# jiangzhengkai/mxdetection

Measured on AMD Instinct MI355X. Metric: images/sec (whole node) Faster R-CNN R50-FPN 3x800x1333, higher is better.
Workload: dtype bf16; 1 GPU; Faster R-CNN ResNet-50-FPN bf16 train step, batch 2/GPU, 3x800x1333 (padded 1344); global_batch=2, parallelism=dp1, frozen=stem+C2, frozen BN folded, optimizer=SGD momentum 0.9 wd 1e-4, launch=hipGraph replay, input=resident, wgrad_side_stream=True, rpn_branch_stream=True, grouped_wgrad=True, filter_prefetch_hints=True, params_trainable=41538304

## Files before the change

### mxdetection_amd/csrc/boxes.hip

```cpp
#include "common.h"

namespace mxdet {

__global__ void box_iou_kernel(const float4* __restrict__ a, int64_t na, const float4* __restrict__ b,
                               int64_t nb, float* __restrict__ out) {
  int64_t idx = (int64_t)blockIdx.x * blockDim.x + threadIdx.x;
  if (idx >= na * nb) return;
  int64_t i = idx / nb, j = idx - i * nb;
  float4 p = a[i], q = b[j];
  out[idx] = mxdet_iou(p.x, p.y, p.z, p.w, q.x, q.y, q.z, q.w);
}

__global__ void anchors_kernel(const float* __restrict__ base, int A, int H, int W, int stride,
                               float4* __restrict__ out) {
  int64_t idx = (int64_t)blockIdx.x * blockDim.x + threadIdx.x;
  int64_t total = (int64_t)H * W * A;
  if (idx >= total) return;
  int a = (int)(idx % A);
  int64_t cell = idx / A;
  int x = (int)(cell % W), y = (int)(cell / W);
  float sx = (float)(x * stride), sy = (float)(y * stride);
  float4 o;
  o.x = base[a * 4 + 0] + sx;
  o.y = base[a * 4 + 1] + sy;
  o.z = base[a * 4 + 2] + sx;
  o.w = base[a * 4 + 3] + sy;
  out[idx] = o;
}

__global__ void fpn_level_kernel(const float* __restrict__ rois, int64_t R, int lvl_min, int lvl_max,
                                 int32_t* __restrict__ levels) {
  int64_t i = (int64_t)blockIdx.x * blockDim.x + threadIdx.x;
  if (i >= R) return;
  const float* r = rois + i * 5;
  int k = mxdet_fpn_level(r[1], r[2], r[3], r[4]);
  k = k < lvl_min ? lvl_min : (k > lvl_max ? lvl_max : k);
  levels[i] = k;
}

__global__ void __launch_bounds__(64)
nms_mask_kernel(const float4* __restrict__ boxes, const int32_t* __restrict__ counts, int n_max,
                int nwords_max, float thresh, unsigned long long* __restrict__ mask) {
  const int col_blk = blockIdx.x, row_blk = blockIdx.y, b = blockIdx.z;
  if (col_blk < row_blk) return;
  int n = counts[b];
  n = n > n_max ? n_max : n;
  if (row_blk * 64 >= n || col_blk * 64 >= n) return;
  __shared__ float4 cb[64];
  const int t = threadIdx.x;
  const float4* bx = boxes + (int64_t)b * n_max;
  int cj = col_blk * 64 + t;
  if (cj < n) cb[t] = bx[cj];
  __syncthreads();
  int i = row_blk * 64 + t;
  if (i >= n) return;
  float4 r = bx[i];
  int ncol = n - col_blk * 64;
  ncol = ncol > 64 ? 64 : ncol;
  unsigned long long bits = 0;
  for (int j = 0; j < ncol; ++j) {
    int c = col_blk * 64 + j;
    float4 q = cb[j];
    float v = mxdet_iou(r.x, r.y, r.z, r.w, q.x, q.y, q.z, q.w);
    if (c > i && v > thresh) bits |= (1ull << j);
  }
  mask[((int64_t)b * n_max + i) * nwords_max + col_blk] = bits;
}

__device__ __forceinline__ unsigned long long readlane64(unsigned long long v, int lane) {
  unsigned lo = (unsigned)v, hi = (unsigned)(v >> 32);
  lo = (unsigned)__builtin_amdgcn_readlane((int)lo, lane);
  hi = (unsigned)__builtin_amdgcn_readlane((int)hi, lane);
  return ((unsigned long long)hi << 32) | lo;
}

__global__ void __launch_bounds__(64)
nms_scan_kernel(const unsigned long long* __restrict__ mask, const int32_t* __restrict__ counts,
                const uint8_t* __restrict__ invalid, int n_max, int nwords_max, int max_keep,
                int32_t* __restrict__ keep_idx, int32_t* __restrict__ num_keep) {
  __shared__ unsigned long long rem[64];
  const int b = blockIdx.x, lane = threadIdx.x;
  int n = counts[b];
  n = n > n_max ? n_max : n;
  n = __builtin_amdgcn_readfirstlane(n);
  const int nw = (n + 63) >> 6;
  const unsigned long long* m = mask + (int64_t)b * n_max * nwords_max;
  for (int w = 0; w < nw; ++w) {
    int idx = w * 64 + lane;
    bool bad = (idx >= n) || (invalid != nullptr && invalid[(int64_t)b * n_max + idx] != 0);
    unsigned long long bm = __ballot(bad);
    if (lane == 0) rem[w] = bm;
  }
  __syncthreads();
  unsigned long long mykeep = 0;
  unsigned long long diag_next = (nw > 0 && lane < n) ? m[(int64_t)lane * nwords_max] : 0ull;
  for (int w = 0; w < nw; ++w) {
    const unsigned long long diag = diag_next;
    if (w + 1 < nw) {
      int row = (w + 1) * 64 + lane;
      diag_next = (row < n) ? m[(int64_t)row * nwords_max + (w + 1)] : 0ull;
    }
    __syncthreads();
    unsigned long long cur = rem[w];
    cur = readlane64(cur, 0);
    unsigned long long keepbits = 0;
    for (int bb = 0; bb < 64; ++bb) {
      unsigned long long d = readlane64(diag, bb);
      if (!((cur >> bb) & 1ull)) {
        keepbits |= (1ull << bb);
        cur |= d;
      }
    }
    if (lane == w) mykeep = keepbits;
    if ((keepbits >> lane) & 1ull) {
      const unsigned long long* row = m + (int64_t)(w * 64 + lane) * nwords_max;
      for (int j = w + 1; j < nw; ++j) {
        unsigned long long v = row[j];
        if (v) atomicOr(&rem[j], v);
      }
    }
  }
  int cnt = __popcll(mykeep);
  int incl = cnt;
  for (int off = 1; off < 64; off <<= 1) {
    int v = __shfl_up(incl, off);
    if (lane >= off) incl += v;
  }
  int excl = incl - cnt;
  int total = __shfl(incl, 63);
  unsigned long long kb = mykeep;
  int pos = excl;
  while (kb) {
    int bb = __ffsll((long long)kb) - 1;
    kb &= kb - 1;
    if (pos < max_keep) keep_idx[(int64_t)b * n_max + pos] = lane * 64 + bb;
    ++pos;
  }
  if (lane == 0) num_keep[b] = total < max_keep ? total : max_keep;
}

template <int NW>
__global__ void __launch_bounds__(64)
nms_scan_rows_kernel(const unsigned long long* __restrict__ mask, const int32_t* __restrict__ counts,
                     const uint8_t* __restrict__ invalid, int n_max, int nwords_max, int max_keep,
                     int32_t* __restrict__ keep_idx, int32_t* __restrict__ num_keep) {
  __shared__ unsigned long long rows[2][64][NW + 1];
  const int b = blockIdx.x, lane = threadIdx.x;
  int n = counts[b];
  n = n > n_max ? n_max : n;
  n = __builtin_amdgcn_readfirstlane(n);
  const int nw = (n + 63) >> 6;
  const unsigned long long* m = mask + (int64_t)b * n_max * NW;
  unsigned long long myrem = 0ull;
  for (int w = 0; w < nw; ++w) {
    int idx = w * 64 + lane;
    bool bad = (idx >= n) || (invalid != nullptr && invalid[(int64_t)b * n_max + idx] != 0);
    unsigned long long bm = __ballot(bad);
    if (lane == w) myrem = bm;
  }
  unsigned long long nxt[NW];
  auto load_row = [&](unsigned long long (&r)[NW], int w) {
    const unsigned long long* bp = m + (int64_t)(w * 64) * NW + lane;
#pragma unroll
    for (int k = 0; k < NW; ++k) r[k] = bp[k * 64];
  };
  auto stage = [&](const unsigned long long (&r)[NW], int buf, int w) {
    unsigned long long* dst = &rows[buf][lane >> 5][lane & 31];
#pragma unroll
    for (int k = 0; k < NW; ++k) dst[k * 2 * (NW + 1)] = r[k];
  };
  load_row(nxt, 0);
  stage(nxt, 0, 0);
  __syncthreads();
  const int myword = lane < NW ? lane : 0;
  unsigned long long mykeep = 0;
  int buf = 0;
  for (int w = 0; w < nw; ++w) {
#ifndef NMS_ABL_NOLOAD
    if (w + 1 < nw) load_row(nxt, w + 1);
#endif
    const unsigned long long diag = rows[buf][lane][w];
    unsigned long long c = readlane64(myrem, w);
#ifndef NMS_ABL_NOCHAIN
#pragma unroll
    for (int bb = 0; bb < 64; ++bb) {
      unsigned long long d = readlane64(diag, bb);
      c |= ((c >> bb) & 1ull) ? 0ull : d;
    }
#else
    c |= readlane64(diag, 0);
#endif
    const unsigned long long keepbits = ~c;
    if (lane == w) mykeep = keepbits;
    const unsigned klo = __builtin_amdgcn_readfirstlane((unsigned)keepbits);
    const unsigned khi = __builtin_amdgcn_readfirstlane((unsigned)(keepbits >> 32));
    unsigned long long acc = 0ull;
#ifndef NMS_ABL_NOOR
#pragma unroll
#else
    if (klo == 0x12345u)
#endif
    for (int ch = 0; ch < 8; ++ch) {
      const unsigned bits = ((ch < 4 ? klo : khi) >> (8 * (ch & 3))) & 0xffu;
      if (bits == 0u) continue;
      unsigned long long v[8];
#pragma unroll
      for (int t = 0; t < 8; ++t) v[t] = rows[buf][8 * ch + t][myword];
#pragma unroll
      for (int t = 0; t < 8; ++t) acc |= ((bits >> t) & 1u) ? v[t] : 0ull;
    }
    if (lane > w && lane < nw) myrem |= acc;
    if (w + 1 < nw) stage(nxt, buf ^ 1, w + 1);
    __syncthreads();
    buf ^= 1;
  }
  int cnt = __popcll(mykeep);
  int incl = cnt;
  for (int off = 1; off < 64; off <<= 1) {
    int v = __shfl_up(incl, off);
    if (lane >= off) incl += v;
  }
  int excl = incl - cnt;
  int total = __shfl(incl, 63);
  unsigned long long kb = mykeep;
  int pos = excl;
  while (kb) {
    int bb = __ffsll((long long)kb) - 1;
    kb &= kb - 1;
    if (pos < max_keep) keep_idx[(int64_t)b * n_max + pos] = lane * 64 + bb;
    ++pos;
  }
  if (lane == 0) num_keep[b] = total < max_keep ? total : max_keep;
}

}

using namespace mxdet;

extern "C" int mxdet_box_iou(const float* boxes_a, int64_t na, const float* boxes_b, int64_t nb,
                             float* out, mxdet_stream_t stream) {
  clear_error();
  MXDET_REQUIRE(na >= 0 && nb >= 0, MXDET_ESHAPE, "box_iou: negative size");
  if (na == 0 || nb == 0) return MXDET_OK;
  MXDET_REQUIRE(boxes_a && boxes_b && out, MXDET_EINVAL, "box_iou: null pointer");
  int64_t total = na * nb;
  hipLaunchKernelGGL(box_iou_kernel, dim3((unsigned)ceil_div<int64_t>(total, 256)), dim3(256), 0,
                     as_stream(stream), (const float4*)boxes_a, na, (const float4*)boxes_b, nb, out);
  return check_launch("box_iou");
}

extern "C" int mxdet_generate_anchors(const float* base_anchors, int32_t A, int32_t H, int32_t W,
                                      int32_t stride, float* out, mxdet_stream_t stream) {
  clear_error();
  MXDET_REQUIRE(A > 0 && H >= 0 && W >= 0 && stride > 0, MXDET_ESHAPE, "generate_anchors: bad shape");
  int64_t total = (int64_t)H * W * A;
  if (total == 0) return MXDET_OK;
  MXDET_REQUIRE(base_anchors && out, MXDET_EINVAL, "generate_anchors: null pointer");
  hipLaunchKernelGGL(anchors_kernel, dim3((unsigned)ceil_div<int64_t>(total, 256)), dim3(256), 0,
                     as_stream(stream), base_anchors, A, H, W, stride, (float4*)out);
  return check_launch("generate_anchors");
}

extern "C" int mxdet_fpn_level_map(const float* rois, int64_t R, int32_t lvl_min, int32_t lvl_max,
                                   int32_t* levels, mxdet_stream_t stream) {
  clear_error();
  MXDET_REQUIRE(R >= 0 && lvl_min <= lvl_max, MXDET_ESHAPE, "fpn_level_map: bad arguments");
  if (R == 0) return MXDET_OK;
  MXDET_REQUIRE(rois && levels, MXDET_EINVAL, "fpn_level_map: null pointer");
  hipLaunchKernelGGL(fpn_level_kernel, dim3((unsigned)ceil_div<int64_t>(R, 256)), dim3(256), 0,
                     as_stream(stream), rois, R, lvl_min, lvl_max, levels);
  return check_launch("fpn_level_map");
}

extern "C" size_t mxdet_nms_batched_workspace_bytes(int32_t B, int32_t n_max) {
  if (B <= 0 || n_max <= 0) return 0;
  size_t nwords = (size_t)(n_max + 63) / 64;
  if (nwords <= 32) nwords = 32;
  return ((size_t)B * n_max + 64) * nwords * sizeof(unsigned long long);
}

extern "C" int mxdet_nms_batched(const float* boxes, const int32_t* counts, const uint8_t* invalid,
                                 int32_t B, int32_t n_max, float thresh, int32_t max_keep,
                                 int32_t* keep_idx, int32_t* num_keep, void* workspace,
                                 size_t workspace_bytes, mxdet_stream_t stream) {
  clear_error();
  MXDET_REQUIRE(B >= 0 && n_max >= 0, MXDET_ESHAPE, "nms_batched: negative size");
  if (B == 0) return MXDET_OK;
  MXDET_REQUIRE(n_max <= 4096, MXDET_ESHAPE, "nms_batched: n_max %d > 4096 unsupported", n_max);
  MXDET_REQUIRE(counts && num_keep, MXDET_EINVAL, "nms_batched: null pointer");
  if (n_max == 0) {
    hipError_t e = zero_async(num_keep, sizeof(int32_t) * B, as_stream(stream));
    MXDET_REQUIRE(e == hipSuccess, MXDET_EHIP, "nms_batched: memset failed");
    return MXDET_OK;
  }
  MXDET_REQUIRE(boxes && keep_idx, MXDET_EINVAL, "nms_batched: null pointer");
  size_t need = mxdet_nms_batched_workspace_bytes(B, n_max);
  MXDET_REQUIRE(workspace && workspace_bytes >= need, MXDET_EWORKSPACE,
                "nms_batched: workspace %zu < %zu", workspace_bytes, need);
  int nwords = (n_max + 63) / 64;
  const int pitch = nwords <= 32 ? 32 : nwords;
  hipLaunchKernelGGL(nms_mask_kernel, dim3(nwords, nwords, B), dim3(64), 0, as_stream(stream),
                     (const float4*)boxes, counts, n_max, pitch, thresh,
                     (unsigned long long*)workspace);
  if (nwords <= 32)
    hipLaunchKernelGGL(nms_scan_rows_kernel<32>, dim3(B), dim3(64), 0, as_stream(stream),
                       (const unsigned long long*)workspace, counts, invalid, n_max, nwords,
                       max_keep < 0 ? 0 : max_keep, keep_idx, num_keep);
  else
    hipLaunchKernelGGL(nms_scan_kernel, dim3(B), dim3(64), 0, as_stream(stream),
                       (const unsigned long long*)workspace, counts, invalid, n_max, nwords,
                       max_keep < 0 ? 0 : max_keep, keep_idx, num_keep);
  return check_launch("nms_batched");
}
```

### mxdetection_amd/csrc/proposal.hip

```cpp
#include "common.h"
#include "select.h"

namespace mxdet {

constexpr int kMaxPre = 4096;

struct PyramidDev {
  int num_levels, A, dtype;
  int H[8], W[8], stride[8];
  const void* cls[8];
  const void* reg[8];
  long long cls_sn[8], cls_sy[8], cls_sx[8], cls_sa[8];
  long long reg_sn[8], reg_sy[8], reg_sx[8], reg_sc[8];
  const float* base[8];
  long long level_offset[8];
  int classes;
};

__device__ __forceinline__ float pyr_score(const PyramidDev& p, int l, int n, int local) {
  int A = p.A;
  int a = local % A;
  int cell = local / A;
  int x = cell % p.W[l], y = cell / p.W[l];
  long long off = n * p.cls_sn[l] + y * p.cls_sy[l] + x * p.cls_sx[l] + a * p.cls_sa[l];
// ... 40 lines not shown
      wave_scan_bins(sd.hist + ((size_t)ps * sd.B + b) * 256, st.remaining, &bin, &cum, &bc, &tot);
      if (bin == 256) { st.all = 1; break; }
      st.prefix |= (unsigned)bin << shift;
      st.mask |= 255u << shift;
      st.remaining -= cum;
      st.eq_count = bc;
    }
    if (threadIdx.x == 0) *sh = st;
  }
  __syncthreads();
  return *sh;
}

__global__ void __launch_bounds__(256)
proposal_hist_kernel(PyramidDev p, long long A_total, const unsigned* __restrict__ fkeys, SelDev sd, int pass) {
  __shared__ unsigned h[256];
  __shared__ SelState sh;
  const int l = blockIdx.y, n = blockIdx.z;
  const int nl = p.H[l] * p.W[l] * p.A;
  const int c0 = blockIdx.x * kSelChunk;
  if (c0 >= nl) return;
  const int b = n * p.num_levels + l;
  h[threadIdx.x] = 0u;
  SelState st = sel_resolve(sd, b, pass, &sh);
  if (st.all) return;
  const unsigned* fk_l = fkeys + (long long)n * A_total + p.level_offset[l];
  const int shift = 24 - 8 * pass;
  const int c1 = c0 + kSelChunk < nl ? c0 + kSelChunk : nl;
  for (int i0 = c0 + threadIdx.x; i0 < c1; i0 += 4 * 256) {
    unsigned kv[4];
#pragma unroll
    for (int u = 0; u < 4; ++u) {
      int i = i0 + u * 256;
      kv[u] = i < c1 ? (~fk_l[i]) & sd.keymask : 0u;
    }
#pragma unroll
    for (int u = 0; u < 4; ++u)
      hist_add_agg(h, (i0 + u * 256 < c1) && (kv[u] & st.mask) == st.prefix, (kv[u] >> shift) & 255u);
  }
  __syncthreads();
  unsigned v = h[threadIdx.x];
  if (v) atomicAdd(&sd.hist[((size_t)pass * sd.B + b) * 256 + threadIdx.x], v);
}

__global__ void __launch_bounds__(256)
proposal_select_kernel(PyramidDev p, long long A_total, const unsigned* __restrict__ fkeys, SelDev sd,
                       unsigned long long* __restrict__ keys) {
  __shared__ SelState sh;
  const int l = blockIdx.y, n = blockIdx.z;
  const int nl = p.H[l] * p.W[l] * p.A;
  const int c0 = blockIdx.x * kSelChunk;
  if (c0 >= nl) return;
  const int b = n * p.num_levels + l;
  const SelState st = sel_resolve(sd, b, sd.npass, &sh);
  const bool split_ties = !st.all && st.remaining < st.eq_count;
  const unsigned goff = (unsigned)p.level_offset[l];
  const unsigned* fk_l = fkeys + (long long)n * A_total + p.level_offset[l];
  unsigned* ties = sd.ties + (long long)n * A_total + p.level_offset[l];
  unsigned long long* out = keys + (long long)b * sd.pre_n;
  const int c1 = c0 + kSelChunk < nl ? c0 + kSelChunk : nl;
  __shared__ unsigned long long s_take[kSelChunk];
  __shared__ unsigned s_tie[kSelChunk];
  __shared__ int s_nt, s_ni, s_bt, s_bi;
  if (threadIdx.x == 0) { s_nt = 0; s_ni = 0; }
  __syncthreads();
  for (int i = c0 + (int)threadIdx.x; i < c1; i += 256) {
    const unsigned fk = fk_l[i];
    const unsigned kv = (~fk) & sd.keymask;
    if (st.all || kv < st.prefix || (kv == st.prefix && !split_ties))
      s_take[atomicAdd(&s_nt, 1)] = ((unsigned long long)fk << 32) | (unsigned long long)(0xffffffffu - (goff + (unsigned)i));
    else if (split_ties && kv == st.prefix)
      s_tie[atomicAdd(&s_ni, 1)] = (unsigned)i;
  }
  __syncthreads();
  if (threadIdx.x == 0) {
    s_bt = s_nt ? atomicAdd(&sd.cnt[b * 2 + 0], s_nt) : 0;
    s_bi = s_ni ? atomicAdd(&sd.cnt[b * 2 + 1], s_ni) : 0;
  }
  __syncthreads();
  for (int j = threadIdx.x; j < s_nt; j += 256) out[s_bt + j] = s_take[j];
  for (int j = threadIdx.x; j < s_ni; j += 256) ties[s_bi + j] = s_tie[j];
}

__global__ void __launch_bounds__(1024)
proposal_finish_kernel(PyramidDev p, long long A_total, const unsigned* __restrict__ fkeys, SelDev sd, int Kpad,
                       unsigned long long* __restrict__ keys, int32_t* __restrict__ counts) {
  __shared__ SelectSmem sm;
  __shared__ SelState sh;
  __shared__ unsigned long long list[kMaxPre];
  __shared__ int n_sel;
  const int l = blockIdx.x, n = blockIdx.y;
  const int b = n * p.num_levels + l;
  const SelState st = sel_resolve(sd, b, sd.npass, &sh);
  const bool split_ties = !st.all && st.remaining < st.eq_count;
  const int got = sd.cnt[b * 2 + 0], n_tie = sd.cnt[b * 2 + 1];
  unsigned long long* out = keys + (long long)b * sd.pre_n;
  for (int i = threadIdx.x; i < Kpad; i += blockDim.x) list[i] = i < got ? out[i] : 0ull;
  if (threadIdx.x == 0) n_sel = got;
  __syncthreads();
  if (split_ties) {
    const unsigned goff = (unsigned)p.level_offset[l];
    const unsigned* fk_l = fkeys + (long long)n * A_total + p.level_offset[l];
    const unsigned* ties = sd.ties + (long long)n * A_total + p.level_offset[l];
    const unsigned T = st.prefix;
    auto tkey = [&](int, unsigned& kv) -> bool { kv = T; return true; };
    auto tidx = [&](int i) -> unsigned { return ties[i]; };
    const unsigned IT = block_tie_threshold(n_tie, st.remaining, T, tkey, tidx, sm);
    for (int j = threadIdx.x; j < n_tie; j += blockDim.x) {
      unsigned i = ties[j];
      if (i <= IT) {
        int pos = atomicAdd(&n_sel, 1);
        list[pos] = ((unsigned long long)fk_l[i] << 32) | (unsigned long long)(0xffffffffu - (goff + i));
      }
    }
    __syncthreads();
  }
  block_bitonic_sort_desc(list, Kpad);
  const int cnt = n_sel;
  for (int i = threadIdx.x; i < sd.pre_n; i += blockDim.x) out[i] = list[i];
  if (threadIdx.x == 0) counts[b] = cnt;
}

__global__ void proposal_decode_kernel(PyramidDev p, int N, int pre_n, const float* __restrict__ im_info,
                                       float min_size, const unsigned long long* __restrict__ keys,
                                       const int32_t* __restrict__ counts, float4* __restrict__ boxes,
                                       uint8_t* __restrict__ invalid) {
  int idx = blockIdx.x * blockDim.x + threadIdx.x;
  int B = N * p.num_levels;
  if (idx >= B * pre_n) return;
  int b = idx / pre_n, j = idx - b * pre_n;
  int n = b / p.num_levels, l = b - n * p.num_levels;
  if (j >= counts[b]) {
    boxes[idx] = make_float4(0.f, 0.f, 0.f, 0.f);
    invalid[idx] = 1;
    return;
  }
  unsigned long long key = keys[idx];
  unsigned gidx = 0xffffffffu - (unsigned)(key & 0xffffffffull);
  int local = (int)(gidx - (unsigned)p.level_offset[l]);
  int A = p.A;
  int a = local % A;
  int cell = local / A;
  int x = cell % p.W[l], y = cell / p.W[l];
  a /= p.classes;
  const float* base = p.base[l] + a * 4;
  float sx = (float)(x * p.stride[l]), sy = (float)(y * p.stride[l]);
  float ax1 = base[0] + sx, ay1 = base[1] + sy, ax2 = base[2] + sx, ay2 = base[3] + sy;
  long long off = n * p.reg_sn[l] + y * p.reg_sy[l] + x * p.reg_sx[l];
  float d0 = load_as_f32(p.reg[l], off + (a * 4 + 0) * p.reg_sc[l], p.dtype);
  float d1 = load_as_f32(p.reg[l], off + (a * 4 + 1) * p.reg_sc[l], p.dtype);
  float d2 = load_as_f32(p.reg[l], off + (a * 4 + 2) * p.reg_sc[l], p.dtype);
  float d3 = load_as_f32(p.reg[l], off + (a * 4 + 3) * p.reg_sc[l], p.dtype);
  float o[4];
  mxdet_decode_clip(ax1, ay1, ax2, ay2, d0, d1, d2, d3, im_info[n * 3 + 0], im_info[n * 3 + 1], o);
  float ms = min_size * im_info[n * 3 + 2];
  float w = o[2] - o[0] + 1.0f, h = o[3] - o[1] + 1.0f;
  boxes[idx] = make_float4(o[0], o[1], o[2], o[3]);
  invalid[idx] = (w < ms || h < ms) ? 1 : 0;
}

__global__ void __launch_bounds__(1024)
proposal_merge_kernel(int L, int pre_n, int lvl_cap, int post_n,
                      const unsigned long long* __restrict__ keys,
                      const float4* __restrict__ boxes, const int32_t* __restrict__ keep_idx,
                      const int32_t* __restrict__ num_keep, float* __restrict__ rois,
                      float* __restrict__ roi_scores, int32_t* __restrict__ roi_anchor,
                      int32_t* __restrict__ num_rois) {
  extern __shared__ __attribute__((aligned(16))) unsigned char smem_raw[];
  unsigned long long* lk = (unsigned long long*)smem_raw;
  __shared__ int nk[8];
  const int n = blockIdx.y, l_own = blockIdx.x;
  if (threadIdx.x < L) {
    int v = num_keep[n * L + threadIdx.x];
    nk[threadIdx.x] = v > lvl_cap ? lvl_cap : v;
  }
  __syncthreads();
  int total = 0;
  for (int l = 0; l < L; ++l) total += nk[l];
  for (int l = 0; l < L; ++l) {
    int b = n * L + l;
    for (int j = threadIdx.x; j < nk[l]; j += blockDim.x)
      lk[l * lvl_cap + j] = keys[(long long)b * pre_n + keep_idx[(long long)b * pre_n + j]];
  }
  __syncthreads();
  {
    const int l = l_own;
    int b = n * L + l;
    for (int j = threadIdx.x; j < nk[l]; j += blockDim.x) {
      unsigned long long e = lk[l * lvl_cap + j];
      int rank = j;
      for (int l2 = 0; l2 < L; ++l2) {
        if (l2 == l) continue;
        int lo = 0, hi = nk[l2];
        const unsigned long long* q = lk + l2 * lvl_cap;
        while (lo < hi) {
          int mid = (lo + hi) >> 1;
          if (q[mid] > e) lo = mid + 1; else hi = mid;
        }
        rank += lo;
      }
      if (rank < post_n) {
        int pos = keep_idx[(long long)b * pre_n + j];
        float4 bx = boxes[(long long)b * pre_n + pos];
        float* r = rois + ((long long)n * post_n + rank) * 5;
        r[0] = (float)n; r[1] = bx.x; r[2] = bx.y; r[3] = bx.z; r[4] = bx.w;
        unsigned fk = (unsigned)(e >> 32);
        unsigned u = (fk & 0x80000000u) ? (fk & 0x7fffffffu) : ~fk;
        roi_scores[(long long)n * post_n + rank] = __uint_as_float(u);
        roi_anchor[(long long)n * post_n + rank] = (int32_t)(0xffffffffu - (unsigned)(e & 0xffffffffull));
      }
    }
  }
  if (l_own != 0) return;
  int nout = total < post_n ? total : post_n;
  for (int j = nout + threadIdx.x; j < post_n; j += blockDim.x) {
    float* r = rois + ((long long)n * post_n + j) * 5;
    r[0] = (float)n; r[1] = 0.f; r[2] = 0.f; r[3] = 0.f; r[4] = 0.f;
    roi_scores[(long long)n * post_n + j] = 0.f;
    roi_anchor[(long long)n * post_n + j] = -1;
  }
  if (threadIdx.x == 0) num_rois[n] = nout;
}

struct ProposalWs {
  unsigned* fkeys;
  unsigned* hist;
  int* cnt;
  unsigned* ties;
  unsigned long long* keys;
  int32_t* counts;
  float4* boxes;
  uint8_t* invalid;
  int32_t* keep_idx;
  int32_t* num_keep;
  void* nms_ws;
  size_t nms_bytes;
  size_t total;
};

static ProposalWs carve(void* base, int B, int pre_n, int N, long long A_total) {
  ProposalWs w;
// ... 18 lines not shown
  w.nms_ws = (void*)(p + take(w.nms_bytes));
  w.total = off;
  return w;
}

}

using namespace mxdet;

extern "C" size_t mxdet_proposal_workspace_bytes(const mxdet_pyramid_t* p, int32_t N,
                                                 int32_t pre_nms_top_n) {
  if (!p || N <= 0 || pre_nms_top_n <= 0 || p->num_levels <= 0) return 0;
  long long At = 0;
  for (int l = 0; l < p->num_levels; ++l) At += (long long)p->H[l] * p->W[l] * p->A;
  return carve(nullptr, N * p->num_levels, pre_nms_top_n, N, At).total;
}

extern "C" int mxdet_proposal(const mxdet_pyramid_t* p, int32_t N, const float* im_info,
                              int32_t pre_nms_top_n, int32_t post_nms_top_n, float nms_thresh,
                              float min_size, float* rois, float* roi_scores, int32_t* roi_anchor,
                              int32_t* num_rois, void* workspace, size_t workspace_bytes,
                              mxdet_stream_t stream) {
  clear_error();
  MXDET_REQUIRE(p != nullptr, MXDET_EINVAL, "proposal: null pyramid");
  MXDET_REQUIRE(N > 0 && p->num_levels > 0 && p->num_levels <= 8 && p->A > 0, MXDET_ESHAPE,
                "proposal: bad N/levels/A");
  MXDET_REQUIRE(pre_nms_top_n > 0 && pre_nms_top_n <= kMaxPre, MXDET_ESHAPE,
                "proposal: pre_nms_top_n %d outside (0,%d]", pre_nms_top_n, kMaxPre);
  MXDET_REQUIRE(post_nms_top_n > 0 && post_nms_top_n <= pre_nms_top_n * p->num_levels, MXDET_ESHAPE,
                "proposal: bad post_nms_top_n %d", post_nms_top_n);
  MXDET_REQUIRE(p->dtype == MXDET_DTYPE_F32 || p->dtype == MXDET_DTYPE_BF16, MXDET_EINVAL,
                "proposal: bad dtype");
  MXDET_REQUIRE(im_info && rois && roi_scores && roi_anchor && num_rois, MXDET_EINVAL,
                "proposal: null pointer");
  const int L = p->num_levels, B = N * L;
  long long A_total = 0;
  for (int l = 0; l < L; ++l) A_total += (long long)p->H[l] * p->W[l] * p->A;
  ProposalWs w = carve(workspace, B, pre_nms_top_n, N, A_total);
  MXDET_REQUIRE(workspace && workspace_bytes >= w.total, MXDET_EWORKSPACE,
                "proposal: workspace %zu < %zu", workspace_bytes, w.total);
  int per_level_post = post_nms_top_n < pre_nms_top_n ? post_nms_top_n : pre_nms_top_n;
  size_t merge_lds = (size_t)L * per_level_post * 8;
  MXDET_REQUIRE(merge_lds <= 150 * 1024, MXDET_ESHAPE, "proposal: levels*post_nms_top_n too large");
  PyramidDev d;
  memset(&d, 0, sizeof(d));
  d.num_levels = L; d.A = p->A; d.dtype = p->dtype;
  d.classes = p->classes > 1 ? p->classes : 1;
  MXDET_REQUIRE(p->A % d.classes == 0, MXDET_ESHAPE, "proposal: A=%d is not a multiple of classes=%d", p->A, d.classes);
  long long off = 0;
  for (int l = 0; l < L; ++l) {
    MXDET_REQUIRE(p->H[l] > 0 && p->W[l] > 0 && p->stride[l] > 0 && p->cls[l] && p->reg[l] &&
                      p->base_anchors[l],
                  MXDET_EINVAL, "proposal: level %d incomplete", l);
    MXDET_REQUIRE((long long)p->H[l] * p->W[l] * p->A < (1ll << 30), MXDET_ESHAPE,
                  "proposal: level %d too large", l);
    d.H[l] = p->H[l]; d.W[l] = p->W[l]; d.stride[l] = p->stride[l];
    d.cls[l] = p->cls[l]; d.reg[l] = p->reg[l];
    d.cls_sn[l] = p->cls_sn[l]; d.cls_sy[l] = p->cls_sy[l]; d.cls_sx[l] = p->cls_sx[l]; d.cls_sa[l] = p->cls_sa[l];
    d.reg_sn[l] = p->reg_sn[l]; d.reg_sy[l] = p->reg_sy[l]; d.reg_sx[l] = p->reg_sx[l]; d.reg_sc[l] = p->reg_sc[l];
    d.base[l] = p->base_anchors[l];
    d.level_offset[l] = off;
    off += (long long)p->H[l] * p->W[l] * p->A;
  }
  int Kpad = 1;
  while (Kpad < pre_nms_top_n) Kpad <<= 1;
  hipStream_t s = as_stream(stream);
  SelDev sd;
  sd.hist = w.hist; sd.cnt = w.cnt; sd.ties = w.ties;
  sd.npass = (p->dtype == MXDET_DTYPE_BF16) ? 2 : 4;
  sd.keymask = (p->dtype == MXDET_DTYPE_BF16) ? 0xffff0000u : 0xffffffffu;
  sd.B = B; sd.pre_n = pre_nms_top_n;
  int max_nl = 0;
  for (int l = 0; l < L; ++l) max_nl = max_nl > p->H[l] * p->W[l] * p->A ? max_nl : p->H[l] * p->W[l] * p->A;
  long long gthreads = (long long)N * A_total;
  if (gthreads < (long long)kMaxPasses * B * 256) gthreads = (long long)kMaxPasses * B * 256;
  hipLaunchKernelGGL(proposal_gather_kernel, dim3((unsigned)ceil_div<long long>(gthreads, 256)), dim3(256), 0, s, d,
                     N, A_total, w.fkeys, sd);
  const dim3 sel_grid(ceil_div(max_nl, kSelChunk), L, N);
  for (int ps = 0; ps < sd.npass; ++ps)
    hipLaunchKernelGGL(proposal_hist_kernel, sel_grid, dim3(256), 0, s, d, A_total, (const unsigned*)w.fkeys, sd, ps);
  hipLaunchKernelGGL(proposal_select_kernel, sel_grid, dim3(256), 0, s, d, A_total, (const unsigned*)w.fkeys, sd,
                     w.keys);
  hipLaunchKernelGGL(proposal_finish_kernel, dim3(L, N), dim3(1024), 0, s, d, A_total, (const unsigned*)w.fkeys, sd,
                     Kpad, w.keys, w.counts);
  int tot = B * pre_nms_top_n;
  hipLaunchKernelGGL(proposal_decode_kernel, dim3(ceil_div(tot, 256)), dim3(256), 0, s, d, N,
                     pre_nms_top_n, im_info, min_size, w.keys, w.counts, w.boxes, w.invalid);
  int rc = check_launch("proposal(topk/decode)");
  if (rc) return rc;
  rc = mxdet_nms_batched((const float*)w.boxes, w.counts, w.invalid, B, pre_nms_top_n, nms_thresh,
                         per_level_post, w.keep_idx, w.num_keep, w.nms_ws, w.nms_bytes, stream);
  if (rc) return rc;
  hipLaunchKernelGGL(proposal_merge_kernel, dim3(L, N), dim3(1024), merge_lds, s, L, pre_nms_top_n,
                     per_level_post, post_nms_top_n, w.keys, w.boxes, w.keep_idx, w.num_keep, rois, roi_scores,
                     roi_anchor, num_rois);
  return check_launch("proposal(merge)");
}
```

### mxdetection_amd/csrc/targets.hip

```cpp
#include "common.h"
#include "select.h"

namespace mxdet {

__global__ void __launch_bounds__(256)
anchor_iou_kernel(const float4* __restrict__ anchors, long long A_total, const float* __restrict__ gt,
                  int G_max, const float* __restrict__ im_info, float allowed_border,
                  float* __restrict__ max_iou, int32_t* __restrict__ argmax,
                  unsigned* __restrict__ gt_max) {
  extern __shared__ __attribute__((aligned(16))) unsigned char smem_raw[];
  float* sg = (float*)smem_raw;
  unsigned* sgm = (unsigned*)(sg + G_max * 5);
  const int n = blockIdx.y;
  for (int i = threadIdx.x; i < G_max * 5; i += blockDim.x) sg[i] = gt[(long long)n * G_max * 5 + i];
  for (int i = threadIdx.x; i < G_max; i += blockDim.x) sgm[i] = 0u;
  __syncthreads();
  long long a = (long long)blockIdx.x * blockDim.x + threadIdx.x;
  if (a < A_total) {
    float4 b = anchors[a];
    float im_h = im_info[n * 3 + 0], im_w = im_info[n * 3 + 1];
    bool inside = (b.x >= -allowed_border) && (b.y >= -allowed_border) &&
                  (b.z < im_w + allowed_border) && (b.w < im_h + allowed_border);
    float best = -1.0f;
    int bi = -1;
// ... 118 lines not shown
  if (inside) {
    key = mxdet_sample_key(seed, step, image_offset + (unsigned)n, 1u, (unsigned)a);
    labels[(long long)n * A_total + a] = 0;
    max_iou[(long long)n * A_total + a] = 0.0f;
    keys[(long long)n * A_total + a] = key;
  }
  if (cand.count != nullptr) cand_append(cand, n, inside ? 0 : -1, key, (int)a);
}

struct AnchorSel { unsigned T[2], IT[2]; int mode[2]; };

__global__ void __launch_bounds__(1024)
anchor_sample_kernel(long long A_total, int batch_size, int max_fg, const int32_t* __restrict__ labels,
                     const unsigned* __restrict__ keys, CandLists cand, AnchorSel* __restrict__ sel) {
  __shared__ SelectSmem sm;
  const int n = blockIdx.x;
  const int32_t* lab = labels + (long long)n * A_total;
  const unsigned* key = keys + (long long)n * A_total;
  const int A = (int)A_total;
  const int n_fg_list = cand.count[n * 4 + 0], n_bg_list = cand.count[n * 4 + 1];
  const int n_fg_all = n_fg_list;
  const unsigned* fk = cand.key + ((long long)n * 2 + 0) * kCandCap;
  const unsigned* bk = cand.key + ((long long)n * 2 + 1) * kCandCap;
  const int* fi = cand.idx + ((long long)n * 2 + 0) * kCandCap;
  const int* bi = cand.idx + ((long long)n * 2 + 1) * kCandCap;
  SelectResult rf, rb;
  if (n_fg_list <= kCandCap) {
    auto kf = [&](int i, unsigned& kv) -> bool { kv = fk[i]; return true; };
    auto xf = [&](int i) -> unsigned { return (unsigned)fi[i]; };
    rf = block_select_threshold(n_fg_list, max_fg, 32, kf, sm, xf);
  } else {
    auto kf = [&](int i, unsigned& kv) -> bool { kv = key[i]; return lab[i] == 1; };
    rf = block_select_threshold(A, max_fg, 32, kf, sm);
  }
  const int nfg = n_fg_all < max_fg ? n_fg_all : max_fg;
  const int want_bg = batch_size - nfg;
  if (n_bg_list <= kCandCap && n_bg_list >= want_bg) {
    auto kb = [&](int i, unsigned& kv) -> bool { kv = bk[i]; return true; };
    auto xb = [&](int i) -> unsigned { return (unsigned)bi[i]; };
    rb = block_select_threshold(n_bg_list, want_bg, 32, kb, sm, xb);
    if (rb.mode == 1) { rb.mode = 0; rb.T = kBgKeyCut - 1u; rb.IT = 0xffffffffu; }
  } else {
    auto kb = [&](int i, unsigned& kv) -> bool { kv = key[i]; return lab[i] == 0; };
    rb = block_select_threshold(A, want_bg, 32, kb, sm);
  }
  if (threadIdx.x == 0) {
    AnchorSel o;
    o.T[0] = rf.T; o.IT[0] = rf.IT; o.mode[0] = rf.mode;
    o.T[1] = rb.T; o.IT[1] = rb.IT; o.mode[1] = rb.mode;
    sel[n] = o;
  }
}

__global__ void __launch_bounds__(256)
anchor_encode_kernel(const float4* __restrict__ anchors, long long A_total, const float* __restrict__ gt,
                     int G_max, int32_t* __restrict__ labels, const int32_t* __restrict__ argmax,
                     const unsigned* __restrict__ keys, const AnchorSel* __restrict__ sel,
                     float4* __restrict__ targets) {
  const int n = blockIdx.y;
  long long a = (long long)blockIdx.x * blockDim.x + threadIdx.x;
  if (a >= A_total) return;
  long long idx = (long long)n * A_total + a;
  int lab = labels[idx];
  if (sel != nullptr && lab >= 0) {
    const AnchorSel s = sel[n];
    const int st = lab == 1 ? 0 : 1;
    SelectResult r;
    r.T = s.T[st]; r.IT = s.IT[st]; r.mode = s.mode[st]; r.n_cand = 0;
    if (!r.chosen(keys[idx], (unsigned)a)) {
      lab = -1;
      labels[idx] = -1;
    }
  }
  float4 t = make_float4(0.f, 0.f, 0.f, 0.f);
  if (lab == 1) {
    int g = argmax[idx];
    float4 b = anchors[a];
    const float* q = gt + ((long long)n * G_max + g) * 5;
    float o[4];
    mxdet_encode(b.x, b.y, b.z, b.w, q[0], q[1], q[2], q[3], o);
    t = make_float4(o[0], o[1], o[2], o[3]);
  }
  targets[idx] = t;
}

__global__ void __launch_bounds__(1024)
proposal_target_kernel(const float* __restrict__ rois, const int32_t* __restrict__ num_rois,
                       int rois_stride, const float* __restrict__ gt, int G_max, int R, int max_fg,
                       float fg_thresh, float bg_hi, float bg_lo, int num_classes, int class_agnostic,
                       float4 means, float4 stds, unsigned seed, unsigned step,
                       const unsigned* __restrict__ step_dev, unsigned image_offset,
                       float* __restrict__ out_rois, int32_t* __restrict__ labels,
                       float* __restrict__ bbox_targets, float* __restrict__ bbox_weights,
                       int32_t* __restrict__ matched_gt, int32_t* __restrict__ num_fg_out) {
  extern __shared__ __attribute__((aligned(16))) unsigned char smem_raw[];
  const int ncap = rois_stride + G_max;
  float* sg = (float*)smem_raw;
  int* vg = (int*)(sg + G_max * 5);
  short* cgt = (short*)(vg + G_max);
  signed char* cstate = (signed char*)(cgt + ((ncap + 7) & ~7));
  __shared__ SelectSmem sm;
  __shared__ int n_valid_gt, cnt_bg;
  const int n = blockIdx.x;
  const unsigned image = image_offset + (unsigned)n;
  if (step_dev) step = *step_dev;
  for (int i = threadIdx.x; i < G_max * 5; i += blockDim.x) sg[i] = gt[(long long)n * G_max * 5 + i];
  if (threadIdx.x == 0) cnt_bg = 0;
  __syncthreads();
  if (threadIdx.x == 0) {
    int c = 0;
    for (int g = 0; g < G_max; ++g)
      if (sg[g * 5 + 4] >= 0.0f) vg[c++] = g;
    n_valid_gt = c;
  }
  __syncthreads();
  int nr = num_rois[n];
  nr = nr > rois_stride ? rois_stride : (nr < 0 ? 0 : nr);
  const int nv = n_valid_gt;
  const int nc = nr + nv;
  const float* rb = rois + (long long)n * rois_stride * 5;
  auto cand_box = [&](int i, float* b) {
    if (i < nr) {
      const float* r = rb + (long long)i * 5;
      b[0] = r[1]; b[1] = r[2]; b[2] = r[3]; b[3] = r[4];
    } else {
      const float* q = sg + vg[i - nr] * 5;
      b[0] = q[0]; b[1] = q[1]; b[2] = q[2]; b[3] = q[3];
    }
  };
  for (int i = threadIdx.x; i < nc; i += blockDim.x) {
    float b[4];
    cand_box(i, b);
    float best = -1.0f;
    int bi = -1;
    for (int k = 0; k < nv; ++k) {
      const float* q = sg + vg[k] * 5;
      float v = mxdet_iou(b[0], b[1], b[2], b[3], q[0], q[1], q[2], q[3]);
      if (v > best) { best = v; bi = vg[k]; }
    }
    if (nv == 0) best = 0.0f;
    signed char st = 0;
    if (best >= fg_thresh && bi >= 0) st = 1;
    else if (best < bg_hi && best >= bg_lo) st = 2;
    cstate[i] = st;
    cgt[i] = (short)bi;
  }
  __syncthreads();
  auto kfg = [&](int i, unsigned& kv) -> bool {
    kv = mxdet_sample_key(seed, step, image, 2u, (unsigned)i);
    return cstate[i] == 1;
  };
  auto kbg = [&](int i, unsigned& kv) -> bool {
    kv = mxdet_sample_key(seed, step, image, 3u, (unsigned)i);
    return cstate[i] == 2;
  };
  SelectResult sel_f = block_select_threshold(nc, max_fg, 32, kfg, sm);
  const int nfg = sel_f.n_cand < max_fg ? sel_f.n_cand : max_fg;
  SelectResult sel_b = block_select_threshold(nc, R - nfg, 32, kbg, sm);
  const int want_bg = (R - nfg) > 0 ? (R - nfg) : 0;
  if (threadIdx.x == 0) cnt_bg = sel_b.n_cand < want_bg ? sel_b.n_cand : want_bg;
  for (int i = threadIdx.x; i < nc; i += blockDim.x) {
    unsigned kv;
    if (cstate[i] == 1) { kfg(i, kv); if (sel_f.chosen(kv, (unsigned)i)) cstate[i] = 3; }
    else if (cstate[i] == 2) { kbg(i, kv); if (sel_b.chosen(kv, (unsigned)i)) cstate[i] = 4; }
  }
  __syncthreads();
// ... 82 lines not shown

using namespace mxdet;

extern "C" size_t mxdet_anchor_target_workspace_bytes(int32_t N, int64_t A_total, int32_t G_max) {
  if (N <= 0 || A_total <= 0 || G_max <= 0) return 0;
  return carve_anchor(nullptr, N, A_total, G_max).total;
}

extern "C" int mxdet_anchor_target(const float* anchors, int64_t A_total, const float* gt_boxes,
                                   int32_t N, int32_t G_max, const float* im_info, float fg_thresh,
                                   float bg_thresh, float allowed_border, int32_t batch_size,
                                   float fg_fraction, uint32_t seed, uint32_t step,
                                   const uint32_t* step_dev, uint32_t image_offset, int32_t* labels,
                                   int32_t* matched_gt,
                                   float* bbox_targets, float* max_iou, void* workspace,
                                   size_t workspace_bytes, mxdet_stream_t stream) {
  clear_error();
  MXDET_REQUIRE(N > 0 && A_total > 0 && G_max > 0, MXDET_ESHAPE, "anchor_target: bad sizes");
  MXDET_REQUIRE(A_total < (1ll << 30) && G_max <= 1024, MXDET_ESHAPE, "anchor_target: too large");
  MXDET_REQUIRE(anchors && gt_boxes && im_info && labels && bbox_targets, MXDET_EINVAL,
                "anchor_target: null pointer");
  AnchorWs w = carve_anchor(workspace, N, A_total, G_max);
  MXDET_REQUIRE(workspace && workspace_bytes >= w.total, MXDET_EWORKSPACE,
                "anchor_target: workspace %zu < %zu", workspace_bytes, w.total);
  hipStream_t s = as_stream(stream);
  int32_t* amax = matched_gt ? matched_gt : w.argmax;
  float* miou = max_iou ? max_iou : w.max_iou;
  hipError_t e = zero_async(w.gt_max, (size_t)N * G_max * 4, s);
  MXDET_REQUIRE(e == hipSuccess, MXDET_EHIP, "anchor_target: memset failed");
  e = zero_async(w.cand.count, w.cand_count_bytes, s);
  MXDET_REQUIRE(e == hipSuccess, MXDET_EHIP, "anchor_target: memset failed");
  CandLists cl = w.cand;
  if (batch_size <= 0) cl.count = nullptr;
  dim3 grid((unsigned)ceil_div<long long>(A_total, 256), N);
  size_t lds = (size_t)G_max * 6 * 4;
  hipLaunchKernelGGL(anchor_iou_kernel, grid, dim3(256), lds, s, (const float4*)anchors,
                     (long long)A_total, gt_boxes, G_max, im_info, allowed_border, miou, amax,
                     w.gt_max);
  hipLaunchKernelGGL(anchor_label_kernel, grid, dim3(256), lds, s, (const float4*)anchors,
                     (long long)A_total, gt_boxes, G_max, miou, w.gt_max, fg_thresh, bg_thresh, seed,
                     step, step_dev, image_offset, labels, w.keys, cl);
  hipLaunchKernelGGL(anchor_nogt_kernel, grid, dim3(256), 0, s, (const float4*)anchors,
                     (long long)A_total, gt_boxes, G_max, im_info, allowed_border, seed, step, step_dev,
                     image_offset, labels, miou, w.keys, cl);
  if (batch_size > 0) {
    int max_fg = (int)(fg_fraction * (float)batch_size);
    hipLaunchKernelGGL(anchor_sample_kernel, dim3(N), dim3(1024), 0, s, (long long)A_total,
                       batch_size, max_fg, (const int32_t*)labels, (const unsigned*)w.keys, cl, w.sel);
  }
  hipLaunchKernelGGL(anchor_encode_kernel, grid, dim3(256), 0, s, (const float4*)anchors,
                     (long long)A_total, gt_boxes, G_max, labels, amax, (const unsigned*)w.keys,
                     batch_size > 0 ? (const AnchorSel*)w.sel : (const AnchorSel*)nullptr,
                     (float4*)bbox_targets);
  return check_launch("anchor_target");
}

extern "C" int mxdet_proposal_target(const float* rois, const int32_t* num_rois, int32_t rois_stride,
                                     const float* gt_boxes, int32_t N, int32_t G_max,
                                     int32_t rois_per_image, float fg_fraction, float fg_thresh,
                                     float bg_hi, float bg_lo, int32_t num_classes,
                                     int32_t class_agnostic, const float* means, const float* stds,
                                     uint32_t seed, uint32_t step, const uint32_t* step_dev,
                                     uint32_t image_offset, float* out_rois, int32_t* labels,
                                     float* bbox_targets,
                                     float* bbox_weights, int32_t* matched_gt, int32_t* num_fg,
                                     mxdet_stream_t stream) {
  clear_error();
  MXDET_REQUIRE(N > 0 && rois_stride > 0 && G_max > 0 && rois_per_image > 0 && num_classes > 0,
                MXDET_ESHAPE, "proposal_target: bad sizes");
  MXDET_REQUIRE(rois && num_rois && gt_boxes && means && stds && out_rois && labels && bbox_targets &&
                    bbox_weights && matched_gt && num_fg,
                MXDET_EINVAL, "proposal_target: null pointer");
  MXDET_REQUIRE(G_max <= 1024 && rois_stride <= 16384, MXDET_ESHAPE, "proposal_target: too large");
  int ncap = rois_stride + G_max;
  size_t lds = (size_t)G_max * 5 * 4 + (size_t)G_max * 4 + (size_t)((ncap + 7) & ~7) * 2 +
               (size_t)((ncap + 15) & ~15);
  MXDET_REQUIRE(lds <= 120 * 1024, MXDET_ESHAPE, "proposal_target: LDS budget exceeded");
  int max_fg = (int)(fg_fraction * (float)rois_per_image);
  float4 m = make_float4(means[0], means[1], means[2], means[3]);
  float4 sd = make_float4(stds[0], stds[1], stds[2], stds[3]);
  {
    const size_t reg_dim = class_agnostic ? 4 : 4 * (size_t)num_classes;
    const size_t bytes = (size_t)N * rois_per_image * reg_dim * sizeof(float);
    hipError_t e = zero_async(bbox_targets, bytes, as_stream(stream));
    if (e == hipSuccess) e = zero_async(bbox_weights, bytes, as_stream(stream));
    MXDET_REQUIRE(e == hipSuccess, MXDET_EHIP, "proposal_target: zero fill failed");
  }
  hipLaunchKernelGGL(proposal_target_kernel, dim3(N), dim3(1024), lds, as_stream(stream), rois,
                     num_rois, rois_stride, gt_boxes, G_max, rois_per_image, max_fg, fg_thresh, bg_hi,
                     bg_lo, num_classes, class_agnostic, m, sd, seed, step, step_dev, image_offset, out_rois,
                     labels, bbox_targets, bbox_weights, matched_gt, num_fg);
  return check_launch("proposal_target");
}
```

Before: 455.0 images/sec.

## Fuse proposal decode into finish, compact NMS mask grid, early-exit scan, merge zero fills

The NMS mask kernel now launches only upper-triangular block pairs, packs four waves per workgroup, and maps a linear index to a (row, col) pair. The NMS scan stops once max_keep boxes have been kept. Proposal decode is folded into the finish kernel, and the two bbox zero fills become one kernel. Together these cut launches and idle blocks in the small RPN/ROI kernels. Risks: the early break leaves later keep words unset, and the float sqrt pair mapping needs its correction loops to stay exact.

```diff
diff --git a/mxdetection_amd/csrc/boxes.hip b/mxdetection_amd/csrc/boxes.hip
--- a/mxdetection_amd/csrc/boxes.hip
+++ b/mxdetection_amd/csrc/boxes.hip
@@ -38,29 +38,44 @@
   levels[i] = k;
 }
 
-__global__ void __launch_bounds__(64)
-nms_mask_kernel(const float4* __restrict__ boxes, const int32_t* __restrict__ counts, int n_max,
+constexpr int kNmsMaskWaves = 4;
+
+__device__ __forceinline__ void nms_tri_pair(int p, int nw, int* row, int* col) {
+  const float t = (float)(2 * nw + 1);
+  int r = (int)((t - sqrtf(t * t - 8.0f * (float)p)) * 0.5f);
+  r = r < 0 ? 0 : (r > nw - 1 ? nw - 1 : r);
+  while (r > 0 && r * nw - r * (r - 1) / 2 > p) --r;
+  while (r + 1 < nw && (r + 1) * nw - (r + 1) * r / 2 <= p) ++r;
+  *row = r;
+  *col = r + (p - (r * nw - r * (r - 1) / 2));
+}
+
+__global__ void __launch_bounds__(kNmsMaskWaves * 64)
+nms_mask_kernel(const float4* __restrict__ boxes, const int32_t* __restrict__ counts, int n_max, int nw_grid,
                 int nwords_max, float thresh, unsigned long long* __restrict__ mask) {
-  const int col_blk = blockIdx.x, row_blk = blockIdx.y, b = blockIdx.z;
-  if (col_blk < row_blk) return;
+  __shared__ float4 cb[kNmsMaskWaves][64];
+  const int t = threadIdx.x & 63, wv = threadIdx.x >> 6;
+  const int b = blockIdx.y;
+  const int pair = blockIdx.x * kNmsMaskWaves + wv;
   int n = counts[b];
   n = n > n_max ? n_max : n;
-  if (row_blk * 64 >= n || col_blk * 64 >= n) return;
-  __shared__ float4 cb[64];
-  const int t = threadIdx.x;
+  int row_blk = 0, col_blk = 0;
+  const bool in_tri = pair < nw_grid * (nw_grid + 1) / 2;
+  if (in_tri) nms_tri_pair(pair, nw_grid, &row_blk, &col_blk);
+  const bool active = in_tri && col_blk * 64 < n;
   const float4* bx = boxes + (int64_t)b * n_max;
-  int cj = col_blk * 64 + t;
-  if (cj < n) cb[t] = bx[cj];
+  const int cj = col_blk * 64 + t;
+  if (active && cj < n) cb[wv][t] = bx[cj];
   __syncthreads();
-  int i = row_blk * 64 + t;
-  if (i >= n) return;
+  const int i = row_blk * 64 + t;
+  if (!active || i >= n) return;
   float4 r = bx[i];
   int ncol = n - col_blk * 64;
   ncol = ncol > 64 ? 64 : ncol;
   unsigned long long bits = 0;
   for (int j = 0; j < ncol; ++j) {
     int c = col_blk * 64 + j;
-    float4 q = cb[j];
+    float4 q = cb[wv][j];
     float v = mxdet_iou(r.x, r.y, r.z, r.w, q.x, q.y, q.z, q.w);
     if (c > i && v > thresh) bits |= (1ull << j);
   }
@@ -174,7 +189,7 @@
   __syncthreads();
   const int myword = lane < NW ? lane : 0;
   unsigned long long mykeep = 0;
-  int buf = 0;
+  int buf = 0, nkept = 0;
   for (int w = 0; w < nw; ++w) {
 #ifndef NMS_ABL_NOLOAD
     if (w + 1 < nw) load_row(nxt, w + 1);
@@ -192,6 +207,8 @@
 #endif
     const unsigned long long keepbits = ~c;
     if (lane == w) mykeep = keepbits;
+    nkept += __popcll(keepbits);
+    if (nkept >= max_keep) break;
     const unsigned klo = __builtin_amdgcn_readfirstlane((unsigned)keepbits);
     const unsigned khi = __builtin_amdgcn_readfirstlane((unsigned)(keepbits >> 32));
     unsigned long long acc = 0ull;
@@ -299,9 +316,10 @@
                 "nms_batched: workspace %zu < %zu", workspace_bytes, need);
   int nwords = (n_max + 63) / 64;
   const int pitch = nwords <= 32 ? 32 : nwords;
-  hipLaunchKernelGGL(nms_mask_kernel, dim3(nwords, nwords, B), dim3(64), 0, as_stream(stream),
-                     (const float4*)boxes, counts, n_max, pitch, thresh,
-                     (unsigned long long*)workspace);
+  MXDET_REQUIRE(B <= 65535, MXDET_ESHAPE, "nms_batched: B %d > 65535 unsupported", B);
+  hipLaunchKernelGGL(nms_mask_kernel, dim3(ceil_div(nwords * (nwords + 1) / 2, kNmsMaskWaves), B),
+                     dim3(kNmsMaskWaves * 64), 0, as_stream(stream), (const float4*)boxes, counts, n_max, nwords, pitch,
+                     thresh, (unsigned long long*)workspace);
   if (nwords <= 32)
     hipLaunchKernelGGL(nms_scan_rows_kernel<32>, dim3(B), dim3(64), 0, as_stream(stream),
                        (const unsigned long long*)workspace, counts, invalid, n_max, nwords,
diff --git a/mxdetection_amd/csrc/proposal.hip b/mxdetection_amd/csrc/proposal.hip
--- a/mxdetection_amd/csrc/proposal.hip
+++ b/mxdetection_amd/csrc/proposal.hip
@@ -146,60 +146,14 @@
   for (int j = threadIdx.x; j < s_ni; j += 256) ties[s_bi + j] = s_tie[j];
 }
 
-__global__ void __launch_bounds__(1024)
-proposal_finish_kernel(PyramidDev p, long long A_total, const unsigned* __restrict__ fkeys, SelDev sd, int Kpad,
-                       unsigned long long* __restrict__ keys, int32_t* __restrict__ counts) {
-  __shared__ SelectSmem sm;
-  __shared__ SelState sh;
-  __shared__ unsigned long long list[kMaxPre];
-  __shared__ int n_sel;
-  const int l = blockIdx.x, n = blockIdx.y;
-  const int b = n * p.num_levels + l;
-  const SelState st = sel_resolve(sd, b, sd.npass, &sh);
-  const bool split_ties = !st.all && st.remaining < st.eq_count;
-  const int got = sd.cnt[b * 2 + 0], n_tie = sd.cnt[b * 2 + 1];
-  unsigned long long* out = keys + (long long)b * sd.pre_n;
-  for (int i = threadIdx.x; i < Kpad; i += blockDim.x) list[i] = i < got ? out[i] : 0ull;
-  if (threadIdx.x == 0) n_sel = got;
-  __syncthreads();
-  if (split_ties) {
-    const unsigned goff = (unsigned)p.level_offset[l];
-    const unsigned* fk_l = fkeys + (long long)n * A_total + p.level_offset[l];
-    const unsigned* ties = sd.ties + (long long)n * A_total + p.level_offset[l];
-    const unsigned T = st.prefix;
-    auto tkey = [&](int, unsigned& kv) -> bool { kv = T; return true; };
-    auto tidx = [&](int i) -> unsigned { return ties[i]; };
-    const unsigned IT = block_tie_threshold(n_tie, st.remaining, T, tkey, tidx, sm);
-    for (int j = threadIdx.x; j < n_tie; j += blockDim.x) {
-      unsigned i = ties[j];
-      if (i <= IT) {
-        int pos = atomicAdd(&n_sel, 1);
-        list[pos] = ((unsigned long long)fk_l[i] << 32) | (unsigned long long)(0xffffffffu - (goff + i));
-      }
-    }
-    __syncthreads();
-  }
-  block_bitonic_sort_desc(list, Kpad);
-  const int cnt = n_sel;
-  for (int i = threadIdx.x; i < sd.pre_n; i += blockDim.x) out[i] = list[i];
-  if (threadIdx.x == 0) counts[b] = cnt;
-}
-
-__global__ void proposal_decode_kernel(PyramidDev p, int N, int pre_n, const float* __restrict__ im_info,
-                                       float min_size, const unsigned long long* __restrict__ keys,
-                                       const int32_t* __restrict__ counts, float4* __restrict__ boxes,
-                                       uint8_t* __restrict__ invalid) {
-  int idx = blockIdx.x * blockDim.x + threadIdx.x;
-  int B = N * p.num_levels;
-  if (idx >= B * pre_n) return;
-  int b = idx / pre_n, j = idx - b * pre_n;
-  int n = b / p.num_levels, l = b - n * p.num_levels;
-  if (j >= counts[b]) {
-    boxes[idx] = make_float4(0.f, 0.f, 0.f, 0.f);
-    invalid[idx] = 1;
+__device__ __forceinline__ void proposal_decode_one(const PyramidDev& p, int n, int l, bool valid, unsigned long long key,
+                                                    const float* __restrict__ im_info, float min_size,
+                                                    float4* __restrict__ box, uint8_t* __restrict__ invalid) {
+  if (!valid) {
+    *box = make_float4(0.f, 0.f, 0.f, 0.f);
+    *invalid = 1;
     return;
   }
-  unsigned long long key = keys[idx];
   unsigned gidx = 0xffffffffu - (unsigned)(key & 0xffffffffull);
   int local = (int)(gidx - (unsigned)p.level_offset[l]);
   int A = p.A;
@@ -219,8 +173,54 @@
   mxdet_decode_clip(ax1, ay1, ax2, ay2, d0, d1, d2, d3, im_info[n * 3 + 0], im_info[n * 3 + 1], o);
   float ms = min_size * im_info[n * 3 + 2];
   float w = o[2] - o[0] + 1.0f, h = o[3] - o[1] + 1.0f;
-  boxes[idx] = make_float4(o[0], o[1], o[2], o[3]);
-  invalid[idx] = (w < ms || h < ms) ? 1 : 0;
+  *box = make_float4(o[0], o[1], o[2], o[3]);
+  *invalid = (w < ms || h < ms) ? 1 : 0;
+}
+
+__global__ void __launch_bounds__(1024)
+proposal_finish_kernel(PyramidDev p, long long A_total, const unsigned* __restrict__ fkeys, SelDev sd, int Kpad,
+                       unsigned long long* __restrict__ keys, int32_t* __restrict__ counts,
+                       const float* __restrict__ im_info, float min_size, float4* __restrict__ boxes,
+                       uint8_t* __restrict__ invalid) {
+  __shared__ SelectSmem sm;
+  __shared__ SelState sh;
+  __shared__ unsigned long long list[kMaxPre];
+  __shared__ int n_sel;
+  const int l = blockIdx.x, n = blockIdx.y;
+  const int b = n * p.num_levels + l;
+  const SelState st = sel_resolve(sd, b, sd.npass, &sh);
+  const bool split_ties = !st.all && st.remaining < st.eq_count;
+  const int got = sd.cnt[b * 2 + 0], n_tie = sd.cnt[b * 2 + 1];
+  unsigned long long* out = keys + (long long)b * sd.pre_n;
+  for (int i = threadIdx.x; i < Kpad; i += blockDim.x) list[i] = i < got ? out[i] : 0ull;
+  if (threadIdx.x == 0) n_sel = got;
+  __syncthreads();
+  if (split_ties) {
+    const unsigned goff = (unsigned)p.level_offset[l];
+    const unsigned* fk_l = fkeys + (long long)n * A_total + p.level_offset[l];
+    const unsigned* ties = sd.ties + (long long)n * A_total + p.level_offset[l];
+    const unsigned T = st.prefix;
+    auto tkey = [&](int, unsigned& kv) -> bool { kv = T; return true; };
+    auto tidx = [&](int i) -> unsigned { return ties[i]; };
+    const unsigned IT = block_tie_threshold(n_tie, st.remaining, T, tkey, tidx, sm);
+    for (int j = threadIdx.x; j < n_tie; j += blockDim.x) {
+      unsigned i = ties[j];
+      if (i <= IT) {
+        int pos = atomicAdd(&n_sel, 1);
+        list[pos] = ((unsigned long long)fk_l[i] << 32) | (unsigned long long)(0xffffffffu - (goff + i));
+      }
+    }
+    __syncthreads();
+  }
+  block_bitonic_sort_desc(list, Kpad);
+  const int cnt = n_sel;
+  for (int i = threadIdx.x; i < sd.pre_n; i += blockDim.x) {
+    const unsigned long long key = list[i];
+    out[i] = key;
+    proposal_decode_one(p, n, l, i < cnt, key, im_info, min_size, boxes + (long long)b * sd.pre_n + i,
+                        invalid + (long long)b * sd.pre_n + i);
+  }
+  if (threadIdx.x == 0) counts[b] = cnt;
 }
 
 __global__ void __launch_bounds__(1024)
@@ -405,10 +405,7 @@
   hipLaunchKernelGGL(proposal_select_kernel, sel_grid, dim3(256), 0, s, d, A_total, (const unsigned*)w.fkeys, sd,
                      w.keys);
   hipLaunchKernelGGL(proposal_finish_kernel, dim3(L, N), dim3(1024), 0, s, d, A_total, (const unsigned*)w.fkeys, sd,
-                     Kpad, w.keys, w.counts);
-  int tot = B * pre_nms_top_n;
-  hipLaunchKernelGGL(proposal_decode_kernel, dim3(ceil_div(tot, 256)), dim3(256), 0, s, d, N,
-                     pre_nms_top_n, im_info, min_size, w.keys, w.counts, w.boxes, w.invalid);
+                     Kpad, w.keys, w.counts, im_info, min_size, w.boxes, w.invalid);
   int rc = check_launch("proposal(topk/decode)");
   if (rc) return rc;
   rc = mxdet_nms_batched((const float*)w.boxes, w.counts, w.invalid, B, pre_nms_top_n, nms_thresh,
diff --git a/mxdetection_amd/csrc/targets.hip b/mxdetection_amd/csrc/targets.hip
--- a/mxdetection_amd/csrc/targets.hip
+++ b/mxdetection_amd/csrc/targets.hip
@@ -224,6 +224,11 @@
     t = make_float4(o[0], o[1], o[2], o[3]);
   }
   targets[idx] = t;
+}
+
+__global__ void zero2_u32_kernel(unsigned* __restrict__ p0, unsigned* __restrict__ p1, long long n) {
+  const long long i = (long long)blockIdx.x * blockDim.x + threadIdx.x;
+  if (i < n) (blockIdx.y ? p1 : p0)[i] = 0u;
 }
 
 __global__ void __launch_bounds__(1024)
@@ -472,9 +477,9 @@
   {
     const size_t reg_dim = class_agnostic ? 4 : 4 * (size_t)num_classes;
     const size_t bytes = (size_t)N * rois_per_image * reg_dim * sizeof(float);
-    hipError_t e = zero_async(bbox_targets, bytes, as_stream(stream));
-    if (e == hipSuccess) e = zero_async(bbox_weights, bytes, as_stream(stream));
-    MXDET_REQUIRE(e == hipSuccess, MXDET_EHIP, "proposal_target: zero fill failed");
+    const long long n4 = (long long)(bytes / 4);
+    hipLaunchKernelGGL(zero2_u32_kernel, dim3((unsigned)((n4 + 255) / 256), 2), dim3(256), 0, as_stream(stream),
+                       (unsigned*)bbox_targets, (unsigned*)bbox_weights, n4);
   }
   hipLaunchKernelGGL(proposal_target_kernel, dim3(N), dim3(1024), lds, as_stream(stream), rois,
                      num_rois, rois_stride, gt_boxes, G_max, rois_per_image, max_fg, fg_thresh, bg_hi,
```

Measured after the change: 453.2 images/sec. About the same (-0.4%).
